# facebookresearch/mbrl-lib

Hardware: AMD Instinct MI355X
Metric: candidate-steps/sec (pop×particles×horizon / plan) per CEM iter; plans/sec (higher is better)
Workload: dtype f32

## Files before the change

mbrl-lib_amd/csrc/cem.hpp:

```cpp
#pragma once
#include <type_traits>

#include "common.hpp"

namespace hipets {

struct CemDev {
    int n_env;
    int pop, H, A, D;
    int K;
    float alpha, one_minus_alpha;
    int return_mean, clipped, unbiased;
    const float* totals = nullptr;
    int P = 0;
    const int* elite_in = nullptr;
};

__device__ __forceinline__ float philox_trunc_normal(uint32_t idx_lo, uint32_t idx_hi, uint64_t seed, uint64_t stream) {
    for (uint32_t attempt = 0; attempt < 64; ++attempt) {
        const Philox4 r = philox4x32_10(idx_lo, idx_hi, attempt, (uint32_t)stream, (uint32_t)seed,
                                        (uint32_t)(seed >> 32) ^ (uint32_t)(stream >> 32) ^ 0x5EED5EEDu);
        float n0, n1, n2, n3;
        box_muller(r.x, r.y, n0, n1);
        if (fabsf(n0) <= 2.0f) return n0;
        if (fabsf(n1) <= 2.0f) return n1;
        box_muller(r.z, r.w, n2, n3);
        if (fabsf(n2) <= 2.0f) return n2;
        if (fabsf(n3) <= 2.0f) return n3;
    }
    return 0.0f;
}

__device__ __forceinline__ float philox_normal(uint32_t idx_lo, uint32_t idx_hi, uint64_t seed, uint64_t stream) {
    const Philox4 r = philox4x32_10(idx_lo, idx_hi, 0u, (uint32_t)stream, (uint32_t)seed,
                                    (uint32_t)(seed >> 32) ^ (uint32_t)(stream >> 32) ^ 0x5EED5EEDu);
    float n0, n1;
    box_muller(r.x, r.y, n0, n1);
    return n0;
}

__global__ void cem_sample_kernel(const CemDev p, const float* __restrict__ mu, const float* __restrict__ disp,
                                  const float* __restrict__ lower, const float* __restrict__ upper,
                                  const float* __restrict__ z_in, unsigned long long seed, unsigned long long stream,
                                  float* __restrict__ population) {
    const long long i = (long long)blockIdx.x * blockDim.x + threadIdx.x;
    if (i >= (long long)p.n_env * p.pop * p.D) return;
    const int d = (int)(i % p.D);
    const int env = (int)(i / ((long long)p.pop * p.D));
    const float m = mu[env * p.D + d], v = disp[env * p.D + d], lb = lower[d], ub = upper[d];
    float x;
    if (p.clipped) {
        const float z = z_in ? z_in[i] : philox_normal((uint32_t)i, (uint32_t)(i >> 32), seed, stream);
        x = m + v * z;
        x = x > lb ? x : lb;
        x = x < ub ? x : ub;
    } else {
        const float lbd = (m - lb) / 2.0f, ubd = (ub - m) / 2.0f;
        const float mv = fminf(lbd * lbd, ubd * ubd);
        const float cv = fminf(mv, v);
        const float z = z_in ? z_in[i] : philox_trunc_normal((uint32_t)i, (uint32_t)(i >> 32), seed, stream);
        x = z * sqrtf(cv) + m;
    }
    population[i] = x;
}

#ifndef HIPETS_REFIT_SKIP
#define HIPETS_REFIT_SKIP 0
#endif
constexpr int kRefitThreads = 1024;
constexpr int kMaxPop = 8192;
constexpr int kRefitScratchBytes = 12288;
constexpr int kSelectMaxK = 1024;
constexpr int kRankSortMax = 640;

__global__ __launch_bounds__(kRefitThreads) void cem_refit_kernel(const CemDev p, float* values, const float* population, float* mu,
                                                                 float* disp, float* best_value, float* best_solution,
                                                                 int* elite_idx_out) {
    extern __shared__ __attribute__((aligned(16))) char smem[];
    {
        const int env = blockIdx.y;
        values += (size_t)env * p.pop;
        if (p.totals && !(HIPETS_REFIT_SKIP & 1)) {
            const float* tot = p.totals + (size_t)env * p.pop * p.P;
            for (int i = threadIdx.x; i < p.pop; i += kRefitThreads) {
                float s = 0.f;
                for (int q0 = 0; q0 < p.P; q0 += 8) {
                    float tv[8];
#pragma unroll
                    for (int u = 0; u < 8; ++u) tv[u] = tot[(size_t)i * p.P + min(q0 + u, p.P - 1)];
#pragma unroll
                    for (int u = 0; u < 8; ++u)
                        if (q0 + u < p.P) s += tv[u];
                }
                values[i] = s / (float)p.P;
            }
        }
        population += (size_t)env * p.pop * p.D;
        mu += (size_t)env * p.D;
        disp += (size_t)env * p.D;
        best_value += env;
        best_solution += (size_t)env * p.D;
        if (elite_idx_out) elite_idx_out += (size_t)env * p.K;
    }
    const int* const elite_in = p.elite_in ? p.elite_in + (size_t)blockIdx.y * p.K : nullptr;
    int n2 = 1;
    while (n2 < p.pop) n2 <<= 1;
    float* key = reinterpret_cast<float*>(smem);
    int* idx = reinterpret_cast<int*>(smem + (size_t)n2 * 4);
    const int tid = threadIdx.x;
    for (int i = tid; i < n2; i += kRefitThreads) {
        float v = -INFINITY;
        if (i < p.pop) {
            v = values[i];
            if (v != v) { v = -1e-10f; values[i] = v; }
        }
        key[i] = v;
        idx[i] = i < p.pop ? i : 0x7FFFFFFF;
    }
    __syncthreads();
    if (elite_in) {
        auto in_range = [&](const int e) { return e < 0 ? 0 : (e >= p.pop ? p.pop - 1 : e); };
        const float top_key = key[in_range(elite_in[0])];
        __syncthreads();
        for (int k = tid; k < p.K; k += kRefitThreads) idx[k] = in_range(elite_in[k]);
        if (tid == 0) key[0] = top_key;
        __syncthreads();
    } else if (HIPETS_REFIT_SKIP & 2) {
    } else if (p.pop <= kRankSortMax) {
        for (int i = tid; i < p.pop; i += kRefitThreads) {
            const float ki = key[i];
            int rank = 0;
#pragma unroll 8
            for (int j = 0; j < i; ++j) rank += key[j] >= ki;
#pragma unroll 8
            for (int j = i + 1; j < p.pop; ++j) rank += key[j] > ki;
            idx[i] = rank;
        }
        __syncthreads();
        int* pos = reinterpret_cast<int*>(smem + (size_t)n2 * 8);
        for (int i = tid; i < p.pop; i += kRefitThreads) pos[idx[i]] = i;
        __syncthreads();
        float top_key = key[pos[0]];
        __syncthreads();
        for (int i = tid; i < p.pop; i += kRefitThreads) idx[i] = pos[i];
        if (tid == 0) key[0] = top_key;
        __syncthreads();
    } else if (p.K <= kSelectMaxK) {
        int* hist = reinterpret_cast<int*>(smem + (size_t)n2 * 8);
        int* ctl = hist + 256;
        int* elist = ctl + 8;
        float* ekey = reinterpret_cast<float*>(elist + kSelectMaxK);
        auto okey = [](float v) {
            const unsigned u = __float_as_uint(v + 0.0f);
            return (u & 0x80000000u) ? ~u : (u | 0x80000000u);
        };
        if (tid == 0) { ctl[0] = 0; ctl[1] = 0; ctl[2] = p.K; ctl[3] = 0; }
        for (int pass = 3; pass >= 0; --pass) {
            for (int b = tid; b < 256; b += kRefitThreads) hist[b] = 0;
            __syncthreads();
            const unsigned prefix = (unsigned)ctl[0], mask = (unsigned)ctl[1];
            for (int i = tid; i < p.pop; i += kRefitThreads) {
                const unsigned u = okey(key[i]);
                if ((u & mask) == prefix) atomicAdd(&hist[(u >> (8 * pass)) & 255u], 1);
            }
            __syncthreads();
            if (tid < 64) {
                const int h0 = hist[4 * tid], h1 = hist[4 * tid + 1], h2 = hist[4 * tid + 2], h3 = hist[4 * tid + 3];
                const int mine = h0 + h1 + h2 + h3;
                int above = mine;
#pragma unroll
                for (int d = 1; d < 64; d <<= 1) {
                    const int o = __shfl_down(above, d, 64);
                    if (tid + d < 64) above += o;
                }
                const int need = ctl[2];
                const int higher = above - mine;
                if (higher < need && need <= above) {
                    int n = need - higher, b = 4 * tid + 3;
                    if (n > h3) { n -= h3; b = 4 * tid + 2;
                        if (n > h2) { n -= h2; b = 4 * tid + 1;
                            if (n > h1) { n -= h1; b = 4 * tid; } } }
                    ctl[0] = (int)(prefix | ((unsigned)b << (8 * pass)));
                    ctl[1] = (int)(mask | (255u << (8 * pass)));
                    ctl[2] = n;
                }
            }
            __syncthreads();
        }
        const unsigned T = (unsigned)ctl[0];
        const int need_eq = ctl[2];
        const bool all_eq = hist[T & 255u] == need_eq;
        for (int i = tid; i < p.pop; i += kRefitThreads) {
            const unsigned u = okey(key[i]);
            bool elite = u > T || (u == T && all_eq);
            if (u == T && !all_eq) {
                int before = 0;
                for (int j = 0; j < i; ++j) before += okey(key[j]) == T;
                elite = before < need_eq;
            }
            if (elite) {
                const int slot = atomicAdd(&ctl[3], 1);
                elist[slot] = i;
                ekey[slot] = key[i];
            }
        }
        __syncthreads();
        int my_pos = -1, my_id = 0;
        float my_key = 0.f;
        if (tid < p.K) {
            my_id = elist[tid];
            my_key = ekey[tid];
            int rank = 0;
            for (int f = 0; f < p.K; ++f) {
                const float kf = ekey[f];
                rank += (kf > my_key) || (kf == my_key && elist[f] < my_id);
            }
            my_pos = rank;
        }
        __syncthreads();
        if (my_pos >= 0) idx[my_pos] = my_id;
        if (my_pos == 0) key[0] = my_key;
        __syncthreads();
    } else
    for (int k = 2; k <= n2; k <<= 1) {
        for (int j = k >> 1; j > 0; j >>= 1) {
            for (int i = tid; i < n2; i += kRefitThreads) {
                const int ixj = i ^ j;
                if (ixj > i) {
                    const float ka = key[i], kb = key[ixj];
                    const int ia = idx[i], ib = idx[ixj];
                    const bool a_first = (ka > kb) || (ka == kb && ia < ib);
                    const bool up = (i & k) == 0;
                    if (up ? !a_first : a_first) {
                        key[i] = kb; key[ixj] = ka;
                        idx[i] = ib; idx[ixj] = ia;
                    }
                }
            }
            __syncthreads();
        }
    }
    if (elite_idx_out && blockIdx.x == 0)
        for (int k = tid; k < p.K; k += kRefitThreads) elite_idx_out[k] = idx[k];

    const float top = key[0];
    const bool improved = blockIdx.x == 0 && top > best_value[0];
    const int top_i = idx[0];
    __syncthreads();

    double* red = reinterpret_cast<double*>(smem + (size_t)n2 * 8);
    const int nb = (int)gridDim.x, bx = (int)blockIdx.x;
    const int Dslice = (((p.D + nb - 1) / nb + 63) / 64) * 64;
    const int d_lo = bx * Dslice, d_hi = min(p.D, d_lo + Dslice);
    int parts = kRefitThreads / Dslice;
    parts = parts < 1 ? 1 : (parts > 8 ? 8 : parts);
    const int G = kRefitThreads / parts;
    const int part = tid / G, dloc = tid % G;
    const int nu = (p.K + parts - 1) / parts;
    auto sweep = [&](const int base, auto nu_tag, auto hold_tag) __attribute__((always_inline)) {
        constexpr int NU = decltype(nu_tag)::value;
        constexpr bool HOLD = decltype(hold_tag)::value;
        const int d = base + dloc;
        const bool live = d < d_hi && part < parts;
        float mu_old = 0.f, disp_old = 0.f;
        float xv[NU];
        double s = 0.0;
        if (live) {
            if (part == 0) { mu_old = mu[d]; disp_old = disp[d]; }
            for (int k0 = part; k0 < (HOLD ? part + 1 : p.K); k0 += parts * NU) {
#pragma unroll
                for (int u = 0; u < NU; ++u) xv[u] = population[(size_t)idx[min(k0 + u * parts, p.K - 1)] * p.D + d];
#pragma unroll
                for (int u = 0; u < NU; ++u)
                    if (k0 + u * parts < p.K) s += (double)xv[u];
            }
        }
        red[tid] = s;
        __syncthreads();
        double mean = 0.0;
        if (live) {
            for (int q = 0; q < parts; ++q) mean += red[q * G + dloc];
            mean /= (double)p.K;
        }
        __syncthreads();
        double ss = 0.0;
        if (live) {
            for (int k0 = part; k0 < (HOLD ? part + 1 : p.K); k0 += parts * NU) {
                if constexpr (!HOLD) {
#pragma unroll
                    for (int u = 0; u < NU; ++u) xv[u] = population[(size_t)idx[min(k0 + u * parts, p.K - 1)] * p.D + d];
                }
#pragma unroll
                for (int u = 0; u < NU; ++u)
                    if (k0 + u * parts < p.K) {
                        const double dv = (double)xv[u] - mean;
                        ss += dv * dv;
                    }
            }
        }
        red[tid] = ss;
        __syncthreads();
        if (live && part == 0) {
            double var = 0.0;
            for (int q = 0; q < parts; ++q) var += red[q * G + dloc];
            var /= (double)(p.unbiased ? (p.K - 1) : p.K);
            const float new_mu = (float)mean;
            const float new_disp = p.clipped ? (float)sqrt(var) : (float)var;
            mu[d] = p.alpha * mu_old + p.one_minus_alpha * new_mu;
            disp[d] = p.alpha * disp_old + p.one_minus_alpha * new_disp;
        }
        __syncthreads();
    };
    constexpr int kBestHold = 4;
    float best_row[kBestHold];
    const bool best_held = p.D <= kBestHold * kRefitThreads;
    if (improved && best_held) {
#pragma unroll
        for (int u = 0; u < kBestHold; ++u) best_row[u] = population[(size_t)top_i * p.D + min(tid + u * kRefitThreads, p.D - 1)];
    }
    for (int base = d_lo; base < ((HIPETS_REFIT_SKIP & 4) ? d_lo : d_hi); base += G) {
        using T = std::true_type;
        using F = std::false_type;
        if (nu <= 2) sweep(base, std::integral_constant<int, 2>{}, T{});
        else if (nu <= 4) sweep(base, std::integral_constant<int, 4>{}, T{});
        else if (nu <= 8) sweep(base, std::integral_constant<int, 8>{}, T{});
        else if (nu <= 16) sweep(base, std::integral_constant<int, 16>{}, T{});
        else sweep(base, std::integral_constant<int, 16>{}, F{});
    }
    if (improved) {
        if (best_held) {
#pragma unroll
            for (int u = 0; u < kBestHold; ++u)
                if (tid + u * kRefitThreads < p.D) best_solution[tid + u * kRefitThreads] = best_row[u];
        } else {
            for (int d = tid; d < p.D; d += kRefitThreads) best_solution[d] = population[(size_t)top_i * p.D + d];
        }
        if (tid == 0) best_value[0] = top;
    }
}

inline int refit_blocks(const int D) { return D <= 128 ? 1 : (D + 127) / 128 > 8 ? 8 : (D + 127) / 128; }

__global__ void cem_init_kernel(const CemDev p, const float* x0, const float* lower, const float* upper, float* mu,
                                float* disp, float* best_value) {
    const int i = blockIdx.x * blockDim.x + threadIdx.x;
    if (i < p.n_env * p.D) {
        const int d = i % p.D;
        mu[i] = x0[i];
        const float w = upper[d] - lower[d];
        disp[i] = p.clipped ? 1.0f : (w * w) / 16.0f;
    }
    if (i < p.n_env) best_value[i] = -INFINITY;
}

}
```

mbrl-lib_amd/csrc/plan.hip:

```cpp
#include <algorithm>
#include <cmath>
#include <vector>

#include "engine.hpp"
#include "lds_optin.hpp"
#include "optim.hpp"

using namespace hipets;

namespace {

int launch_mppi_sample(int n_env, int pop, int H, int A, float beta, const float* mean, const float* past_action, const float* lower, const float* upper,
                       const float* z, uint64_t seed, uint64_t stream_id, float* population, hipStream_t st) {
    const long long npop = (long long)n_env * pop;
    const long long D = (long long)H * A;
    if (D <= kMppiSampleMaxD) {
        const int G = mppi_sample_group(npop, (int)D);
        hipLaunchKernelGGL(mppi_sample_staged_kernel, dim3((unsigned)((npop + G - 1) / G)), dim3(kMppiSampleThreads), (size_t)G * D * 4, st, n_env, pop, H, A, G, beta,
                           mean, past_action, lower, upper, z, (unsigned long long)seed, (unsigned long long)stream_id, population);
    } else {
        const long long n = npop * A;
        hipLaunchKernelGGL(mppi_sample_kernel, dim3((unsigned)((n + 255) / 256)), dim3(256), 0, st, n_env, pop, H, A, beta, mean, past_action, lower, upper, z,
                           (unsigned long long)seed, (unsigned long long)stream_id, population);
    }
    HCHECK(hipGetLastError());
    return 0;
}

int launch_mppi_update(hipets_engine* e, int n_env, int pop, int D, float gamma, float* values, const float* population, float* mean, hipStream_t st) {
    static LdsOptIn once[2];
    HCHECK(full_lds_once(once[0], reinterpret_cast<const void*>(&mppi_update_kernel<kMppiTileMax / 16>), (int)e->lds_max));
    HCHECK(full_lds_once(once[1], reinterpret_cast<const void*>(&mppi_update_kernel<kMppiTileMax / 32>), (int)e->lds_max));
    const int tile_c = mppi_update_tile(pop, e->lds_max);
    const dim3 grid(mppi_update_blocks(D), n_env);
    if (tile_c == kMppiTileMax)
        hipLaunchKernelGGL(mppi_update_kernel<kMppiTileMax / 16>, grid, dim3(kMppiThreads), mppi_update_smem(pop, tile_c), st, pop, D, gamma, values, population, mean);
    else
        hipLaunchKernelGGL(mppi_update_kernel<kMppiTileMax / 32>, grid, dim3(kMppiThreads), mppi_update_smem(pop, tile_c), st, pop, D, gamma, values, population, mean);
    HCHECK(hipGetLastError());
    return 0;
}

int plan_prologue(hipets_engine* e, const float* s0, int n_env, int H, int iters, uint64_t seed, uint64_t first_stream, hipStream_t st) {
    const ModelDev& md = e->md;
    if (e->s0.ensure((size_t)n_env * md.obs_dim * 4)) return 1;
    if (stage_h2d(e, e->s0.p, s0, (size_t)n_env * md.obs_dim * 4, st)) return 1;
    return plan_step_keys(e, H, iters, seed, first_stream, st);
}

inline void shard_bounds(int pop, int world, int r, int* lo, int* hi) {
    const int base = pop / world, extra = pop % world;
    *lo = r * base + std::min(r, extra);
    *hi = *lo + base + (r < extra ? 1 : 0);
}

int trace_iter(hipets_engine* e, int i, int rows, size_t nd, const float* population, const float* values, const float* mu,
               const float* disp, hipStream_t st, int n_env = 1) {
    if (!e->has_trace) return 0;
    const hipets_plan_trace& t = e->trace;
    if (rows > t.max_rows) return fail("plan trace: iteration %d evaluates %d candidates, trace buffers hold %d", i, rows, t.max_rows);
    const size_t ne = (size_t)n_env;
    if (t.populations && population)
        HCHECK(hipMemcpyAsync(t.populations + (size_t)i * t.max_rows * nd, population, (size_t)rows * nd * 4, hipMemcpyDeviceToDevice, st));
    if (t.values && values) HCHECK(hipMemcpyAsync(t.values + (size_t)i * t.max_rows, values, (size_t)rows * 4, hipMemcpyDeviceToDevice, st));
    if (t.mus && mu) HCHECK(hipMemcpyAsync(t.mus + (size_t)i * ne * nd, mu, ne * nd * 4, hipMemcpyDeviceToDevice, st));
    if (t.dispersions && disp) HCHECK(hipMemcpyAsync(t.dispersions + (size_t)i * ne * nd, disp, ne * nd * 4, hipMemcpyDeviceToDevice, st));
    return 0;
}

CemDev make_cem(const hipets_cem_params* p, int n_env = 1) {
    CemDev c{};
    c.n_env = n_env;
    c.pop = p->population_size;
    c.H = p->horizon;
    c.A = p->act_dim;
    c.D = p->horizon * p->act_dim;
    c.K = p->elite_num;
    c.alpha = (float)p->alpha;
    c.one_minus_alpha = (float)(1.0 - (double)p->alpha);
    c.return_mean = p->return_mean_elites;
    c.clipped = p->clipped_normal;
    c.unbiased = p->unbiased_var;
    return c;
}
// ... 27 lines not shown
    const int world = e->comm_world, rank = e->comm_rank;
    int lo, hi;
    shard_bounds(rows, world, rank, &lo, &hi);
    const int width = (rows + world - 1) / world;
    const size_t nd = (size_t)H * e->md.act_dim;
    float* shard_out = world == 1 ? e->values.as<float>() : e->shard_values.as<float>();
    if (le->ok()) le->note(rollout_impl(e, population + (size_t)lo * nd, nullptr, hi - lo, H, P, ro, shard_out, stream));
    if (world > 1) {
        hipStream_t st = reinterpret_cast<hipStream_t>(stream);
        if (comm_all_gather(e, (size_t)width, st)) return 1;
        if (le->ok()) le->note(comm_unpad_shards(e, rows, width, st));
    }
    return 0;
}

struct PlanObjective {
    enum Kind { ENSEMBLE, SHARDED, PLANET } kind = ENSEMBLE;
    const float* s0 = nullptr;
    const float* latent0 = nullptr;
    const float* belief0 = nullptr;

    bool is_planet() const { return kind == PLANET; }
    bool is_sharded() const { return kind == SHARDED; }
    uint64_t rollout_seed(const hipets_engine* e, uint64_t seed) const {
        return seed + (is_sharded() ? (uint64_t)e->comm_rank : 0ull) * 0x9E3779B97F4A7C15ull;
    }
    size_t shard_width(const hipets_engine* e, int max_rows) const { return (size_t)((max_rows + e->comm_world - 1) / e->comm_world); }
    int reserve_shards(hipets_engine* e, int max_rows) const {
        if (!is_sharded()) return 0;
        const size_t width = shard_width(e, max_rows);
        return e->shard_values.ensure(width * 4) || e->gathered.ensure((size_t)e->comm_world * width * 4);
    }
    int clear_padding(hipets_engine* e, int max_rows, hipStream_t st) const {
        if (is_sharded()) HCHECK(hipMemsetAsync(e->shard_values.p, 0, shard_width(e, max_rows) * 4, st));
        return 0;
    }
    void refit_from_totals(hipets_engine* e, CemDev* c, int P) const {
        if (is_sharded()) return;
        c->totals = e->totals.as<float>();
        c->P = P;
    }
    int evaluate(hipets_engine* e, const float* population, int rows, int H, int P, const hipets_rollout_opts* ro, float* returns,
                 void* stream, LocalErr& le) const {
        if (is_sharded()) return sharded_evaluate(e, population, rows, H, P, ro, stream, &le);
        if (!le.ok()) return 0;
        if (!is_planet()) {
            le.note(rollout_impl(e, population, nullptr, rows, H, P, ro, returns, stream));
            return 0;
        }
        hipets_planet_opts po{};
        po.seed = ro->seed;
        po.stream_id = ro->stream_id;
        po.n_env = ro->n_env;
        le.note(planet_rollout_impl(e, population, latent0, belief0, rows, H, P, &po, returns, reinterpret_cast<hipStream_t>(stream)));
        return 0;
    }
};
PlanObjective ensemble_objective(const float* s0, PlanObjective::Kind kind = PlanObjective::ENSEMBLE) {
    PlanObjective o;
    o.kind = kind;
    o.s0 = s0;
    return o;
}
PlanObjective planet_objective(const float* latent0, const float* belief0) {
    PlanObjective o;
    o.kind = PlanObjective::PLANET;
    o.latent0 = latent0;
    o.belief0 = belief0;
    return o;
}

int check_plan(const hipets_engine* e, const PlanObjective& obj, bool args, int A, int n_env, int P) {
    const bool planet = obj.is_planet();
    if (planet && !(e && e->has_planet)) return fail("engine has no PlaNet model (call hipets_planet_set_model)");
    if (!planet && !(e && e->has_model)) return fail("engine has no model (call hipets_set_model)");
    if (!args || (planet ? !(obj.latent0 && obj.belief0) : !obj.s0)) return fail("null argument");
    if (planet && A != e->pd.action) return fail("act_dim %d != model action_size %d", A, e->pd.action);
    if (!planet && A != e->md.act_dim) return fail("act_dim %d != model act_dim %d", A, e->md.act_dim);
    if (n_env < 1 || n_env > 4096) return fail("n_env %d outside [1, 4096]", n_env);
    if (planet && P < 1) return fail("bad pop/horizon/particles");
    return 0;
}

int launch_cem_refit(const CemDev& c, float* values, const float* population, float* mu, float* disp, float* best_value, float* best_solution,
                     int* elite_idx, hipStream_t st) {
    int n2 = 1;
    while (n2 < c.pop) n2 <<= 1;
    hipLaunchKernelGGL(cem_refit_kernel, dim3(refit_blocks(c.D), c.n_env), dim3(kRefitThreads), (size_t)n2 * 8 + kRefitScratchBytes, st, c, values,
                       population, mu, disp, best_value, best_solution, elite_idx);
    HCHECK(hipGetLastError());
    return 0;
}

struct PlanLoop {
    int n_env, H, P, iters;
    uint64_t first_stream, stream_stride, rollout_stream;
    const float* population;
    float* returns;
};
template <class Prologue, class Rows, class Sample, class Refit>
int run_plan(hipets_engine* e, const PlanObjective& obj, const PlanLoop& pl, uint64_t seed, void* stream, Prologue prologue, Rows rows, Sample sample,
             Refit refit) {
    hipets_rollout_opts ro{};
    ro.mode = e->plan_mode;
    ro.seed = obj.rollout_seed(e, seed);
    ro.n_env = pl.n_env;
    const bool carry_on = obj.is_sharded();
    LocalErr le;
    le.note(prologue(ro.seed));
    for (int i = 0; i < pl.iters && (carry_on || le.ok()); ++i) {
        const uint64_t sid = (pl.first_stream + (uint64_t)i) * pl.stream_stride;
        if (le.ok()) le.note(sample(i, sid));
        ro.stream_id = sid + pl.rollout_stream;
        if (obj.evaluate(e, pl.population, rows(i), pl.H, pl.P, &ro, pl.returns, stream, le)) return 1;
        if (le.ok()) le.note(refit(i));
    }
    return le.report();
}

int plan_cem_impl(hipets_engine* e, const hipets_cem_params* p, int32_t n_env, const float* x0, const float* lower, const float* upper,
                  const PlanObjective& obj, int32_t P, uint64_t seed, uint64_t plan_id, float* out, void* stream) {
    if (check_cem(p) || check_plan(e, obj, x0 && lower && upper && out, p->act_dim, n_env, P)) return 1;
    if (obj.is_sharded() && check_shards(e, p->population_size, P)) return 1;
    hipStream_t st = reinterpret_cast<hipStream_t>(stream);
    HCHECK(hipSetDevice(e->device));
    ENTER_STREAM(e, st);
    const CemDev c = make_cem(p, n_env);
    const size_t nd = (size_t)n_env * c.D, npop = (size_t)n_env * c.pop;
    if (e->mu.ensure(nd * 4) || e->disp.ensure(nd * 4) || e->best_solution.ensure(nd * 4) || e->best_value.ensure((size_t)n_env * 4 + 16) ||
        e->population.ensure(npop * c.D * 4) || e->values.ensure(npop * 4) || obj.reserve_shards(e, c.pop))
        return 1;
    const int iters = p->num_iterations;
    const PlanLoop pl{n_env, c.H, P, iters, plan_id * (uint64_t)iters, 1, 0, e->population.as<float>(), nullptr};
    auto prologue = [&](uint64_t rollout_seed) -> int {
        if (obj.clear_padding(e, c.pop, st)) return 1;
        hipLaunchKernelGGL(cem_init_kernel, dim3((unsigned)((nd + 255) / 256)), dim3(256), 0, st, c, x0, lower, upper, e->mu.as<float>(),
                           e->disp.as<float>(), e->best_value.as<float>());
        HCHECK(hipGetLastError());
        HCHECK(hipMemsetAsync(e->best_solution.p, 0, nd * 4, st));
        return obj.is_planet() ? 0 : plan_prologue(e, obj.s0, n_env, c.H, iters, rollout_seed, pl.first_stream, st);
    };
    auto sample = [&](int, uint64_t sid) -> int {
        const long long n = (long long)npop * c.D;
        hipLaunchKernelGGL(cem_sample_kernel, dim3((unsigned)((n + 255) / 256)), dim3(256), 0, st, c, e->mu.as<float>(), e->disp.as<float>(),
                           lower, upper, (const float*)nullptr, (unsigned long long)seed, (unsigned long long)sid, e->population.as<float>());
        HCHECK(hipGetLastError());
        return 0;
    };
    auto refit = [&](int i) -> int {
        int* eidx = (e->has_trace && e->trace.elite_idx) ? e->trace.elite_idx + (size_t)i * n_env * c.K : nullptr;
        CemDev cr = c;
        obj.refit_from_totals(e, &cr, P);
        if (launch_cem_refit(cr, e->values.as<float>(), e->population.as<float>(), e->mu.as<float>(), e->disp.as<float>(), e->best_value.as<float>(),
                             e->best_solution.as<float>(), eidx, st))
            return 1;
        return trace_iter(e, i, (int)npop, (size_t)c.D, e->population.as<float>(), e->values.as<float>(), e->mu.as<float>(), e->disp.as<float>(), st, n_env);
    };
    if (run_plan(e, obj, pl, seed, stream, prologue, [&](int) { return (int)npop; }, sample, refit)) return 1;
    HCHECK(hipMemcpyAsync(out, p->return_mean_elites ? e->mu.p : e->best_solution.p, nd * 4, hipMemcpyDeviceToDevice, st));
    return 0;
}

int plan_mppi_impl(hipets_engine* e, int32_t pop, int32_t H, int32_t A, int32_t num_iterations, double gamma, double beta, int32_t n_env,
                   float* mean, const float* lower, const float* upper, const PlanObjective& obj, int32_t P, uint64_t seed, uint64_t plan_id,
                   void* stream) {
    if (check_plan(e, obj, mean && lower && upper, A, n_env, P)) return 1;
    if (pop < 1 || pop > 12000) return fail("population_size %d outside [1, 12000]", pop);
    if (H < 1 || num_iterations < 0) return fail("bad horizon/num_iterations");
    if (obj.is_sharded() && check_shards(e, pop, P)) return 1;
    hipStream_t st = reinterpret_cast<hipStream_t>(stream);
    HCHECK(hipSetDevice(e->device));
    ENTER_STREAM(e, st);
    const size_t nd = (size_t)H * A, npop = (size_t)n_env * pop;
    if (e->mu.ensure(n_env * nd * 4) || e->past_action.ensure((size_t)n_env * A * 4) || e->population.ensure(npop * nd * 4) ||
        e->values.ensure(npop * 4) || obj.reserve_shards(e, pop))
        return 1;
    const PlanLoop pl{n_env, H, P, num_iterations, plan_id * (uint64_t)num_iterations, 1, 0, e->population.as<float>(), e->values.as<float>()};
    auto prologue = [&](uint64_t rollout_seed) -> int {
        if (obj.clear_padding(e, pop, st)) return 1;
        HCHECK(hipMemcpyAsync(e->mu.p, mean, n_env * nd * 4, hipMemcpyDeviceToDevice, st));
        hipLaunchKernelGGL(mppi_shift_kernel, dim3((unsigned)((n_env * nd + 255) / 256)), dim3(256), 0, st, n_env, H, A, e->mu.as<float>(), mean,
                           e->past_action.as<float>());
        HCHECK(hipGetLastError());
        return obj.is_planet() ? 0 : plan_prologue(e, obj.s0, n_env, H, num_iterations, rollout_seed, pl.first_stream, st);
    };
    auto sample = [&](int, uint64_t sid) -> int {
        return launch_mppi_sample(n_env, pop, H, A, (float)beta, mean, e->past_action.as<float>(), lower, upper, nullptr, seed, sid,
                                  e->population.as<float>(), st);
    };
    auto update = [&](int k) -> int {
        if (launch_mppi_update(e, n_env, pop, (int)nd, (float)gamma, e->values.as<float>(), e->population.as<float>(), mean, st)) return 1;
        return trace_iter(e, k, (int)npop, nd, e->population.as<float>(), e->values.as<float>(), mean, nullptr, st, n_env);
    };
    return run_plan(e, obj, pl, seed, stream, prologue, [&](int) { return (int)npop; }, sample, update);
}

int plan_icem_impl(hipets_engine* e, const hipets_icem_params* p, int32_t n_env, const float* x0, const float* lower, const float* upper,
                   float* elite, int32_t has_elite, const int32_t* keep_idx, const PlanObjective& obj, int32_t P, uint64_t seed, uint64_t plan_id,
                   float* out, void* stream) {
    if (check_plan(e, obj, p && x0 && lower && upper && elite && out, p ? p->act_dim : 0, n_env, P)) return 1;
    if (p->horizon < 2 || p->horizon > kMaxHorizon) return fail("iCEM horizon %d outside [2, %d]", p->horizon, kMaxHorizon);
    const int K = p->elite_num, keep = p->keep_elite_size, iters = p->num_iterations, H = p->horizon, A = p->act_dim;
    if (K < 1 || keep < 0 || keep > K) return fail("elite_num %d / keep_elite_size %d invalid", K, keep);
    if (p->population_size < 1 || iters < 0 || !(p->population_decay_factor > 0.0)) return fail("bad iCEM parameters");
    std::vector<int> sizes(iters), rows_of(iters);
    int max_rows = 1;
    for (int i = 0, he = has_elite; i < iters; ++i, he = 1) {
        int n = (int)std::ceil(std::fmax((double)p->population_size * std::pow(p->population_decay_factor, -(double)i), 2.0 * K));
        const int m = p->population_size_module;
        if (m > 0 && n % m) n += m - n % m;
        sizes[i] = n;
        if (n + keep > kMaxPop) return fail("iCEM iteration %d evaluates %d candidates (max %d)", i, n + keep, kMaxPop);
        rows_of[i] = n + (he ? ((i == iters - 1 && i != 0) ? 1 : keep) : 0);
        if (K > rows_of[i]) return fail("elite_num %d invalid", K);
        max_rows = std::max(max_rows, n + keep);
        if (obj.is_sharded() && check_shards(e, rows_of[i], P)) return 1;
    }
    hipStream_t st = reinterpret_cast<hipStream_t>(stream);
    HCHECK(hipSetDevice(e->device));
    ENTER_STREAM(e, st);
    const size_t nd = (size_t)H * A, ne = (size_t)n_env;
    if (e->mu.ensure(ne * nd * 4) || e->disp.ensure(ne * nd * 4) || e->best_solution.ensure(ne * nd * 4) || e->best_value.ensure(ne * 4 + 16) ||
        e->population.ensure(ne * max_rows * nd * 4) || e->values.ensure(ne * max_rows * 4) ||
        e->kept.ensure(ne * std::max(keep, 1) * nd * 4) || e->elite_idx.ensure(ne * K * 4) || e->keep_idx.ensure(ne * std::max(keep, 1) * 4) ||
        (!obj.is_planet() && e->s0.ensure(ne * e->md.obs_dim * 4)) || obj.reserve_shards(e, max_rows))
        return 1;
    hipets_cem_params cp{};
    cp.population_size = std::max(K, 1);
    cp.horizon = H;
    cp.act_dim = A;
    cp.num_iterations = iters;
    cp.elite_num = K;
    cp.alpha = p->alpha;
    cp.return_mean_elites = p->return_mean_elites;
    cp.clipped_normal = 0;
    cp.unbiased_var = 0;
    float* popbuf = e->population.as<float>();
    const PlanLoop pl{n_env, H, P, iters, plan_id * (uint64_t)iters, 4, 3, popbuf, nullptr};
    auto prologue = [&](uint64_t) -> int {
        if (obj.clear_padding(e, max_rows, st)) return 1;
        hipLaunchKernelGGL(cem_init_kernel, dim3((unsigned)((ne * nd + 255) / 256)), dim3(256), 0, st, make_cem(&cp, n_env), x0, lower, upper,
                           e->mu.as<float>(), e->disp.as<float>(), e->best_value.as<float>());
        HCHECK(hipGetLastError());
        HCHECK(hipMemsetAsync(e->best_solution.p, 0, ne * nd * 4, st));
        return obj.is_planet() ? 0 : stage_h2d(e, e->s0.p, obj.s0, ne * e->md.obs_dim * 4, st);
    };
    auto sample = [&](int i, uint64_t sid) -> int {
        const int n = sizes[i], rows = rows_of[i], extra = rows - n;
        launch_icem_sample(st, n_env, rows, n, H, A, (float)p->colored_noise_exponent, e->mu.as<float>(), e->disp.as<float>(), lower, upper,
                           (const float*)nullptr, (unsigned long long)seed, (unsigned long long)sid, popbuf);
        HCHECK(hipGetLastError());
        if (!extra) return 0;
        float* tail = popbuf + (size_t)n * nd;
        if (i == iters - 1 && i != 0) {
            hipLaunchKernelGGL(icem_append_mu_kernel, dim3((unsigned)((ne * nd + 255) / 256)), dim3(256), 0, st, n_env, rows, n, (int)nd,
                               e->mu.as<float>(), popbuf);
            HCHECK(hipGetLastError());
            return 0;
        }
        const int32_t* kidx = keep_idx ? keep_idx + (size_t)i * n_env * keep : e->keep_idx.as<int32_t>();
        if (!keep_idx) {
            hipLaunchKernelGGL(icem_keep_select_kernel, dim3(n_env), dim3(256), (size_t)K * 8, st, K, keep, (unsigned long long)seed,
                               (unsigned long long)(sid + 2), e->keep_idx.as<int32_t>());
            HCHECK(hipGetLastError());
        }
        const long long ng = (long long)keep * nd;
        if (i == 0) {
            hipLaunchKernelGGL(gather_rows_kernel, dim3((unsigned)((ng + 255) / 256), n_env), dim3(256), 0, st, keep, (int)nd, elite, kidx,
                               e->kept.as<float>(), (long long)K * nd, (long long)keep * nd);
            HCHECK(hipGetLastError());
            hipLaunchKernelGGL(icem_shift_kernel, dim3((unsigned)((ne * ng + 255) / 256)), dim3(256), 0, st, n_env, rows, keep, H, A,
                               e->kept.as<float>(), e->mu.as<float>(), e->disp.as<float>(), (const float*)nullptr,
                               (unsigned long long)seed, (unsigned long long)(sid + 1), tail);
            HCHECK(hipGetLastError());
        } else {
            hipLaunchKernelGGL(gather_rows_kernel, dim3((unsigned)((ng + 255) / 256), n_env), dim3(256), 0, st, keep, (int)nd, elite, kidx,
                               tail, (long long)K * nd, (long long)rows * nd);
            HCHECK(hipGetLastError());
        }
        return 0;
    };
    auto refit = [&](int i) -> int {
        const int rows = rows_of[i];
        cp.population_size = rows;
        if (check_cem(&cp)) return 1;
        CemDev cr = make_cem(&cp, n_env);
        obj.refit_from_totals(e, &cr, P);
        if (launch_cem_refit(cr, e->values.as<float>(), popbuf, e->mu.as<float>(), e->disp.as<float>(), e->best_value.as<float>(),
                             e->best_solution.as<float>(), e->elite_idx.as<int>(), st))
            return 1;
        const long long nk = (long long)K * nd;
        hipLaunchKernelGGL(gather_rows_kernel, dim3((unsigned)((nk + 255) / 256), n_env), dim3(256), 0, st, K, (int)nd, popbuf, e->elite_idx.as<int32_t>(),
                           elite, (long long)rows * nd, (long long)K * nd);
        HCHECK(hipGetLastError());
        if (trace_iter(e, i, n_env * rows, nd, popbuf, e->values.as<float>(), e->mu.as<float>(), e->disp.as<float>(), st, n_env)) return 1;
        if (e->has_trace && e->trace.elite_idx)
            HCHECK(hipMemcpyAsync(e->trace.elite_idx + (size_t)i * n_env * K, e->elite_idx.p, ne * K * 4, hipMemcpyDeviceToDevice, st));
        return 0;
    };
    if (run_plan(e, obj, pl, seed, stream, prologue, [&](int i) { return n_env * rows_of[i]; }, sample, refit)) return 1;
    HCHECK(hipMemcpyAsync(out, p->return_mean_elites ? e->mu.p : e->best_solution.p, ne * nd * 4, hipMemcpyDeviceToDevice, st));
    return 0;
}

}

extern "C" {

int hipets_cem_sample(hipets_engine* e, const hipets_cem_params* p, const float* mu, const float* dispersion,
                      const float* lower, const float* upper, const float* z, uint64_t seed, uint64_t stream_id,
                      float* population, void* stream) {
    if (!e) return fail("null engine");
    if (check_cem(p)) return 1;
    if (!mu || !dispersion || !lower || !upper || !population) return fail("null argument");
    HCHECK(hipSetDevice(e->device));
    const CemDev c = make_cem(p);
    const long long n = (long long)c.pop * c.D;
    hipLaunchKernelGGL(cem_sample_kernel, dim3((unsigned)((n + 255) / 256)), dim3(256), 0, reinterpret_cast<hipStream_t>(stream), c,
                       mu, dispersion, lower, upper, z, (unsigned long long)seed, (unsigned long long)stream_id, population);
    HCHECK(hipGetLastError());
    return 0;
}

int hipets_cem_refit(hipets_engine* e, const hipets_cem_params* p, float* values, const float* population, float* mu,
                     float* dispersion, float* best_value, float* best_solution, int32_t* elite_idx, void* stream) {
    if (!e) return fail("null engine");
    if (check_cem(p)) return 1;
// ... 152 lines not shown
```

Baseline: 290.6 million.

## Fuse CEM refit with next-iteration sampling and wave-ballot rank sort

Adds a fused boundary variant of the CEM refit kernel. It computes particle means inline, updates mu/disp and the best solution per D-slice, then samples the next population, or writes the output on the last iteration, in the same launch. This removes the separate sample kernel, the final memcpy and the memset. The small-population rank sort is replaced with wave-level ballot/popcount counting over register-held keys. best_value is now double-buffered across iterations so blocks can read the previous best without racing. The cost is a wider grid with some redundant per-block sorting and more complex indexing.

```diff
diff --git a/mbrl-lib_amd/csrc/cem.hpp b/mbrl-lib_amd/csrc/cem.hpp
--- a/mbrl-lib_amd/csrc/cem.hpp
+++ b/mbrl-lib_amd/csrc/cem.hpp
@@ -14,6 +14,16 @@
     const float* totals = nullptr;
     int P = 0;
     const int* elite_in = nullptr;
+    int slice = 0, parts = 1;
+};
+
+struct CemNext {
+    const float* lower = nullptr;
+    const float* upper = nullptr;
+    unsigned long long seed = 0, stream = 0;
+    float* next_population = nullptr;
+    float* out = nullptr;
+    const float* best_in = nullptr;
 };
 
 __device__ __forceinline__ float philox_trunc_normal(uint32_t idx_lo, uint32_t idx_hi, uint64_t seed, uint64_t stream) {
@@ -39,15 +49,8 @@
     return n0;
 }
 
-__global__ void cem_sample_kernel(const CemDev p, const float* __restrict__ mu, const float* __restrict__ disp,
-                                  const float* __restrict__ lower, const float* __restrict__ upper,
-                                  const float* __restrict__ z_in, unsigned long long seed, unsigned long long stream,
-                                  float* __restrict__ population) {
-    const long long i = (long long)blockIdx.x * blockDim.x + threadIdx.x;
-    if (i >= (long long)p.n_env * p.pop * p.D) return;
-    const int d = (int)(i % p.D);
-    const int env = (int)(i / ((long long)p.pop * p.D));
-    const float m = mu[env * p.D + d], v = disp[env * p.D + d], lb = lower[d], ub = upper[d];
+__device__ __forceinline__ float cem_sample_one(const CemDev& p, const long long i, const float m, const float v, const float lb, const float ub,
+                                                const float* __restrict__ z_in, unsigned long long seed, unsigned long long stream) {
     float x;
     if (p.clipped) {
         const float z = z_in ? z_in[i] : philox_normal((uint32_t)i, (uint32_t)(i >> 32), seed, stream);
@@ -61,6 +64,18 @@
         const float z = z_in ? z_in[i] : philox_trunc_normal((uint32_t)i, (uint32_t)(i >> 32), seed, stream);
         x = z * sqrtf(cv) + m;
     }
+    return x;
+}
+
+__global__ void cem_sample_kernel(const CemDev p, const float* __restrict__ mu, const float* __restrict__ disp,
+                                  const float* __restrict__ lower, const float* __restrict__ upper,
+                                  const float* __restrict__ z_in, unsigned long long seed, unsigned long long stream,
+                                  float* __restrict__ population) {
+    const long long i = (long long)blockIdx.x * blockDim.x + threadIdx.x;
+    if (i >= (long long)p.n_env * p.pop * p.D) return;
+    const int d = (int)(i % p.D);
+    const int env = (int)(i / ((long long)p.pop * p.D));
+    const float x = cem_sample_one(p, i, mu[env * p.D + d], disp[env * p.D + d], lower[d], upper[d], z_in, seed, stream);
     population[i] = x;
 }
 
@@ -73,28 +88,42 @@
 constexpr int kSelectMaxK = 1024;
 constexpr int kRankSortMax = 640;
 
+__device__ __forceinline__ float particle_mean(const float* __restrict__ row, const int P) {
+    float s = 0.f;
+    if ((P & 3) == 0) {
+        const float4* r4 = reinterpret_cast<const float4*>(row);
+        const int nq = P >> 2;
+        for (int q0 = 0; q0 < nq; q0 += 8) {
+            float4 tv[8];
+#pragma unroll
+            for (int u = 0; u < 8; ++u) tv[u] = r4[min(q0 + u, nq - 1)];
+#pragma unroll
+            for (int u = 0; u < 8; ++u)
+                if (q0 + u < nq) { s += tv[u].x; s += tv[u].y; s += tv[u].z; s += tv[u].w; }
+        }
+    } else {
+        for (int q0 = 0; q0 < P; q0 += 8) {
+            float tv[8];
+#pragma unroll
+            for (int u = 0; u < 8; ++u) tv[u] = row[min(q0 + u, P - 1)];
+#pragma unroll
+            for (int u = 0; u < 8; ++u)
+                if (q0 + u < P) s += tv[u];
+        }
+    }
+    return s / (float)P;
+}
+
+template <bool FUSED>
 __global__ __launch_bounds__(kRefitThreads) void cem_refit_kernel(const CemDev p, float* values, const float* population, float* mu,
                                                                  float* disp, float* best_value, float* best_solution,
-                                                                 int* elite_idx_out) {
+                                                                 int* elite_idx_out, const CemNext nx) {
     extern __shared__ __attribute__((aligned(16))) char smem[];
+    const float* tot = nullptr;
     {
         const int env = blockIdx.y;
         values += (size_t)env * p.pop;
-        if (p.totals && !(HIPETS_REFIT_SKIP & 1)) {
-            const float* tot = p.totals + (size_t)env * p.pop * p.P;
-            for (int i = threadIdx.x; i < p.pop; i += kRefitThreads) {
-                float s = 0.f;
-                for (int q0 = 0; q0 < p.P; q0 += 8) {
-                    float tv[8];
-#pragma unroll
-                    for (int u = 0; u < 8; ++u) tv[u] = tot[(size_t)i * p.P + min(q0 + u, p.P - 1)];
-#pragma unroll
-                    for (int u = 0; u < 8; ++u)
-                        if (q0 + u < p.P) s += tv[u];
-                }
-                values[i] = s / (float)p.P;
-            }
-        }
+        if (p.totals && !(HIPETS_REFIT_SKIP & 1)) tot = p.totals + (size_t)env * p.pop * p.P;
         population += (size_t)env * p.pop * p.D;
         mu += (size_t)env * p.D;
         disp += (size_t)env * p.D;
@@ -111,8 +140,10 @@
     for (int i = tid; i < n2; i += kRefitThreads) {
         float v = -INFINITY;
         if (i < p.pop) {
-            v = values[i];
-            if (v != v) { v = -1e-10f; values[i] = v; }
+            bool fresh = tot != nullptr;
+            v = tot ? particle_mean(tot + (size_t)i * p.P, p.P) : values[i];
+            if (v != v) { v = -1e-10f; fresh = true; }
+            if (fresh && blockIdx.x == 0) values[i] = v;
         }
         key[i] = v;
         idx[i] = i < p.pop ? i : 0x7FFFFFFF;
@@ -127,18 +158,32 @@
         __syncthreads();
     } else if (HIPETS_REFIT_SKIP & 2) {
     } else if (p.pop <= kRankSortMax) {
-        for (int i = tid; i < p.pop; i += kRefitThreads) {
-            const float ki = key[i];
+        constexpr int kBlocks = kRankSortMax / 64;
+        static_assert(kRankSortMax % 64 == 0 && kRankSortMax / (kRefitThreads / 64) <= 64, "rank counting: a wave's elements fit its lanes");
+        const int lane = tid & 63, wave = tid >> 6, nblk = (p.pop + 63) >> 6;
+        float kj[kBlocks];
+#pragma unroll
+        for (int r = 0; r < kBlocks; ++r) kj[r] = 64 * r + lane < n2 ? key[64 * r + lane] : -INFINITY;
+        const int mine = __float_as_int(key[min(wave + (kRefitThreads / 64) * lane, n2 - 1)]);
+        int* pos = reinterpret_cast<int*>(smem + (size_t)n2 * 8);
+        for (int i = wave, t = 0; i < p.pop; i += kRefitThreads / 64, ++t) {
+            const float ki = __int_as_float(__builtin_amdgcn_readlane(mine, t));
+            const int bi = i >> 6;
             int rank = 0;
-#pragma unroll 8
-            for (int j = 0; j < i; ++j) rank += key[j] >= ki;
-#pragma unroll 8
-            for (int j = i + 1; j < p.pop; ++j) rank += key[j] > ki;
-            idx[i] = rank;
-        }
-        __syncthreads();
-        int* pos = reinterpret_cast<int*>(smem + (size_t)n2 * 8);
-        for (int i = tid; i < p.pop; i += kRefitThreads) pos[idx[i]] = i;
+#pragma unroll
+            for (int r = 0; r < kBlocks; ++r) {
+                if (r >= nblk) break;
+                unsigned long long m;
+                if (r < bi) m = __ballot(kj[r] >= ki);
+                else if (r > bi) m = __ballot(kj[r] > ki);
+                else {
+                    const unsigned long long below = (1ull << (i & 63)) - 1ull;
+                    m = (__ballot(kj[r] >= ki) & below) | (__ballot(kj[r] > ki) & ~below);
+                }
+                rank += __popcll(m);
+            }
+            if (lane == 0) pos[rank] = i;
+        }
         __syncthreads();
         float top_key = key[pos[0]];
         __syncthreads();
@@ -244,16 +289,16 @@
         for (int k = tid; k < p.K; k += kRefitThreads) elite_idx_out[k] = idx[k];
 
     const float top = key[0];
-    const bool improved = blockIdx.x == 0 && top > best_value[0];
+    const float best_old = FUSED ? nx.best_in[blockIdx.y] : (blockIdx.x == 0 ? best_value[0] : INFINITY);
+    const bool improved = top > best_old;
     const int top_i = idx[0];
     __syncthreads();
 
     double* red = reinterpret_cast<double*>(smem + (size_t)n2 * 8);
-    const int nb = (int)gridDim.x, bx = (int)blockIdx.x;
-    const int Dslice = (((p.D + nb - 1) / nb + 63) / 64) * 64;
-    const int d_lo = bx * Dslice, d_hi = min(p.D, d_lo + Dslice);
-    int parts = kRefitThreads / Dslice;
-    parts = parts < 1 ? 1 : (parts > 8 ? 8 : parts);
+    const int bx = (int)blockIdx.x;
+    const int d_lo = min(p.D, bx * p.slice), d_hi = min(p.D, d_lo + p.slice);
+    const int parts = p.parts;
+    float* fresh = reinterpret_cast<float*>(smem + (size_t)n2 * 8 + kRefitThreads * 8);
     const int G = kRefitThreads / parts;
     const int part = tid / G, dloc = tid % G;
     const int nu = (p.K + parts - 1) / parts;
@@ -306,17 +351,23 @@
             var /= (double)(p.unbiased ? (p.K - 1) : p.K);
             const float new_mu = (float)mean;
             const float new_disp = p.clipped ? (float)sqrt(var) : (float)var;
-            mu[d] = p.alpha * mu_old + p.one_minus_alpha * new_mu;
-            disp[d] = p.alpha * disp_old + p.one_minus_alpha * new_disp;
+            const float mu_d = p.alpha * mu_old + p.one_minus_alpha * new_mu;
+            const float disp_d = p.alpha * disp_old + p.one_minus_alpha * new_disp;
+            mu[d] = mu_d;
+            disp[d] = disp_d;
+            if constexpr (FUSED) { fresh[2 * (d - d_lo)] = mu_d; fresh[2 * (d - d_lo) + 1] = disp_d; }
         }
         __syncthreads();
     };
     constexpr int kBestHold = 4;
     float best_row[kBestHold];
-    const bool best_held = p.D <= kBestHold * kRefitThreads;
+    const bool best_held = FUSED || p.D <= kBestHold * kRefitThreads;
     if (improved && best_held) {
-#pragma unroll
-        for (int u = 0; u < kBestHold; ++u) best_row[u] = population[(size_t)top_i * p.D + min(tid + u * kRefitThreads, p.D - 1)];
+        if constexpr (FUSED) best_row[0] = population[(size_t)top_i * p.D + min(d_lo + tid, p.D - 1)];
+        else {
+#pragma unroll
+            for (int u = 0; u < kBestHold; ++u) best_row[u] = population[(size_t)top_i * p.D + min(tid + u * kRefitThreads, p.D - 1)];
+        }
     }
     for (int base = d_lo; base < ((HIPETS_REFIT_SKIP & 4) ? d_lo : d_hi); base += G) {
         using T = std::true_type;
@@ -327,7 +378,21 @@
         else if (nu <= 16) sweep(base, std::integral_constant<int, 16>{}, T{});
         else sweep(base, std::integral_constant<int, 16>{}, F{});
     }
-    if (improved) {
+    if constexpr (FUSED) {
+        const int W = d_hi - d_lo, env = (int)blockIdx.y;
+        if (improved && tid < W) best_solution[d_lo + tid] = best_row[0];
+        if (bx == 0 && tid == 0) best_value[0] = improved ? top : best_old;
+        if (nx.out && tid < W)
+            nx.out[(size_t)env * p.D + d_lo + tid] = p.return_mean ? fresh[2 * tid] : (improved ? best_row[0] : best_solution[d_lo + tid]);
+        if (nx.next_population) {
+            float* next = nx.next_population + (size_t)env * p.pop * p.D;
+            for (int e = tid; e < p.pop * W; e += kRefitThreads) {
+                const int c = e / W, dl = e - c * W, d = d_lo + dl;
+                const long long i = ((long long)env * p.pop + c) * p.D + d;
+                next[(size_t)c * p.D + d] = cem_sample_one(p, i, fresh[2 * dl], fresh[2 * dl + 1], nx.lower[d], nx.upper[d], nullptr, nx.seed, nx.stream);
+            }
+        }
+    } else if (improved) {
         if (best_held) {
 #pragma unroll
             for (int u = 0; u < kBestHold; ++u)
@@ -340,17 +405,32 @@
 }
 
 inline int refit_blocks(const int D) { return D <= 128 ? 1 : (D + 127) / 128 > 8 ? 8 : (D + 127) / 128; }
+inline int refit_slice(const int D) { return (((D + refit_blocks(D) - 1) / refit_blocks(D) + 63) / 64) * 64; }
+inline int refit_parts(const int D) {
+    const int parts = kRefitThreads / refit_slice(D);
+    return parts < 1 ? 1 : (parts > 8 ? 8 : parts);
+}
+constexpr int kBoundaryMaxSlice = 128;
+constexpr int kBoundaryWorkgroups = 256;
+static_assert(kRefitThreads * 8 + kBoundaryMaxSlice * 8 <= kRefitScratchBytes, "fused boundary: LDS behind the partial sums");
+inline int boundary_slice(const int D, const int n_env) {
+    const int per_env = kBoundaryWorkgroups / (n_env < 1 ? 1 : n_env) < 1 ? 1 : kBoundaryWorkgroups / (n_env < 1 ? 1 : n_env);
+    const int nb = D < per_env ? D : per_env;
+    const int s = (D + nb - 1) / nb;
+    return s > kBoundaryMaxSlice ? 0 : s;
+}
 
 __global__ void cem_init_kernel(const CemDev p, const float* x0, const float* lower, const float* upper, float* mu,
-                                float* disp, float* best_value) {
+                                float* disp, float* best_value, float* best_solution) {
     const int i = blockIdx.x * blockDim.x + threadIdx.x;
     if (i < p.n_env * p.D) {
         const int d = i % p.D;
         mu[i] = x0[i];
         const float w = upper[d] - lower[d];
         disp[i] = p.clipped ? 1.0f : (w * w) / 16.0f;
-    }
-    if (i < p.n_env) best_value[i] = -INFINITY;
-}
-
-}
+        best_solution[i] = 0.0f;
+    }
+    if (i < 2 * p.n_env) best_value[i] = -INFINITY;
+}
+
+}
diff --git a/mbrl-lib_amd/csrc/plan.hip b/mbrl-lib_amd/csrc/plan.hip
--- a/mbrl-lib_amd/csrc/plan.hip
+++ b/mbrl-lib_amd/csrc/plan.hip
@@ -1,5 +1,6 @@
 #include <algorithm>
 #include <cmath>
+#include <cstdlib>
 #include <vector>
 
 #include "engine.hpp"
@@ -193,12 +194,39 @@
     return 0;
 }
 
-int launch_cem_refit(const CemDev& c, float* values, const float* population, float* mu, float* disp, float* best_value, float* best_solution,
+int launch_cem_refit(CemDev c, float* values, const float* population, float* mu, float* disp, float* best_value, float* best_solution,
                      int* elite_idx, hipStream_t st) {
     int n2 = 1;
     while (n2 < c.pop) n2 <<= 1;
-    hipLaunchKernelGGL(cem_refit_kernel, dim3(refit_blocks(c.D), c.n_env), dim3(kRefitThreads), (size_t)n2 * 8 + kRefitScratchBytes, st, c, values,
-                       population, mu, disp, best_value, best_solution, elite_idx);
+    c.slice = refit_slice(c.D);
+    c.parts = refit_parts(c.D);
+    hipLaunchKernelGGL(cem_refit_kernel<false>, dim3(refit_blocks(c.D), c.n_env), dim3(kRefitThreads), (size_t)n2 * 8 + kRefitScratchBytes, st, c, values,
+                       population, mu, disp, best_value, best_solution, elite_idx, CemNext{});
+    HCHECK(hipGetLastError());
+    return 0;
+}
+
+int plan_boundary_slice(const int D, const int n_env) {
+    static const int forced = [] { const char* v = std::getenv("HIPETS_BOUNDARY_SLICE"); return v && v[0] ? std::atoi(v) : -1; }();
+    if (forced < 0) return boundary_slice(D, n_env);
+    return forced > kBoundaryMaxSlice ? kBoundaryMaxSlice : forced;
+}
+int launch_cem_boundary(CemDev c, int slice, float* values, const float* population, float* mu, float* disp, float* best_out, float* best_solution,
+                        int* elite_idx, const CemNext& nx, hipStream_t st) {
+    int n2 = 1;
+    while (n2 < c.pop) n2 <<= 1;
+    c.slice = slice;
+    c.parts = refit_parts(c.D);
+    hipLaunchKernelGGL(cem_refit_kernel<true>, dim3((c.D + c.slice - 1) / c.slice, c.n_env), dim3(kRefitThreads), (size_t)n2 * 8 + kRefitScratchBytes, st, c,
+                       values, population, mu, disp, best_out, best_solution, elite_idx, nx);
+    HCHECK(hipGetLastError());
+    return 0;
+}
+
+int launch_cem_init(hipets_engine* e, const CemDev& c, const float* x0, const float* lower, const float* upper, hipStream_t st) {
+    const size_t n = std::max((size_t)c.n_env * c.D, (size_t)2 * c.n_env);
+    hipLaunchKernelGGL(cem_init_kernel, dim3((unsigned)((n + 255) / 256)), dim3(256), 0, st, c, x0, lower, upper, e->mu.as<float>(), e->disp.as<float>(),
+                       e->best_value.as<float>(), e->best_solution.as<float>());
     HCHECK(hipGetLastError());
     return 0;
 }
@@ -238,20 +266,19 @@
     ENTER_STREAM(e, st);
     const CemDev c = make_cem(p, n_env);
     const size_t nd = (size_t)n_env * c.D, npop = (size_t)n_env * c.pop;
-    if (e->mu.ensure(nd * 4) || e->disp.ensure(nd * 4) || e->best_solution.ensure(nd * 4) || e->best_value.ensure((size_t)n_env * 4 + 16) ||
+    if (e->mu.ensure(nd * 4) || e->disp.ensure(nd * 4) || e->best_solution.ensure(nd * 4) || e->best_value.ensure((size_t)n_env * 8 + 16) ||
         e->population.ensure(npop * c.D * 4) || e->values.ensure(npop * 4) || obj.reserve_shards(e, c.pop))
         return 1;
     const int iters = p->num_iterations;
     const PlanLoop pl{n_env, c.H, P, iters, plan_id * (uint64_t)iters, 1, 0, e->population.as<float>(), nullptr};
     auto prologue = [&](uint64_t rollout_seed) -> int {
-        if (obj.clear_padding(e, c.pop, st)) return 1;
-        hipLaunchKernelGGL(cem_init_kernel, dim3((unsigned)((nd + 255) / 256)), dim3(256), 0, st, c, x0, lower, upper, e->mu.as<float>(),
-                           e->disp.as<float>(), e->best_value.as<float>());
-        HCHECK(hipGetLastError());
-        HCHECK(hipMemsetAsync(e->best_solution.p, 0, nd * 4, st));
+        if (obj.clear_padding(e, c.pop, st) || launch_cem_init(e, c, x0, lower, upper, st)) return 1;
         return obj.is_planet() ? 0 : plan_prologue(e, obj.s0, n_env, c.H, iters, rollout_seed, pl.first_stream, st);
     };
-    auto sample = [&](int, uint64_t sid) -> int {
+    const int slice = plan_boundary_slice(c.D, n_env);
+    const bool one_launch = slice > 0;
+    auto sample = [&](int i, uint64_t sid) -> int {
+        if (one_launch && i > 0) return 0;
         const long long n = (long long)npop * c.D;
         hipLaunchKernelGGL(cem_sample_kernel, dim3((unsigned)((n + 255) / 256)), dim3(256), 0, st, c, e->mu.as<float>(), e->disp.as<float>(),
                            lower, upper, (const float*)nullptr, (unsigned long long)seed, (unsigned long long)sid, e->population.as<float>());
@@ -262,13 +289,29 @@
         int* eidx = (e->has_trace && e->trace.elite_idx) ? e->trace.elite_idx + (size_t)i * n_env * c.K : nullptr;
         CemDev cr = c;
         obj.refit_from_totals(e, &cr, P);
-        if (launch_cem_refit(cr, e->values.as<float>(), e->population.as<float>(), e->mu.as<float>(), e->disp.as<float>(), e->best_value.as<float>(),
-                             e->best_solution.as<float>(), eidx, st))
+        if (!one_launch) {
+            if (launch_cem_refit(cr, e->values.as<float>(), e->population.as<float>(), e->mu.as<float>(), e->disp.as<float>(), e->best_value.as<float>(),
+                                 e->best_solution.as<float>(), eidx, st))
+                return 1;
+            return trace_iter(e, i, (int)npop, (size_t)c.D, e->population.as<float>(), e->values.as<float>(), e->mu.as<float>(), e->disp.as<float>(), st, n_env);
+        }
+        if (trace_iter(e, i, (int)npop, (size_t)c.D, e->population.as<float>(), nullptr, nullptr, nullptr, st, n_env)) return 1;
+        const bool last = i + 1 == iters;
+        CemNext nx;
+        nx.lower = lower;
+        nx.upper = upper;
+        nx.seed = seed;
+        nx.stream = (pl.first_stream + (uint64_t)i + 1) * pl.stream_stride;
+        nx.next_population = last ? nullptr : e->population.as<float>();
+        nx.out = last ? out : nullptr;
+        nx.best_in = e->best_value.as<float>() + (size_t)(i & 1) * n_env;
+        if (launch_cem_boundary(cr, slice, e->values.as<float>(), e->population.as<float>(), e->mu.as<float>(), e->disp.as<float>(),
+                                e->best_value.as<float>() + (size_t)((i + 1) & 1) * n_env, e->best_solution.as<float>(), eidx, nx, st))
             return 1;
-        return trace_iter(e, i, (int)npop, (size_t)c.D, e->population.as<float>(), e->values.as<float>(), e->mu.as<float>(), e->disp.as<float>(), st, n_env);
+        return trace_iter(e, i, (int)npop, (size_t)c.D, nullptr, e->values.as<float>(), e->mu.as<float>(), e->disp.as<float>(), st, n_env);
     };
     if (run_plan(e, obj, pl, seed, stream, prologue, [&](int) { return (int)npop; }, sample, refit)) return 1;
-    HCHECK(hipMemcpyAsync(out, p->return_mean_elites ? e->mu.p : e->best_solution.p, nd * 4, hipMemcpyDeviceToDevice, st));
+    if (!one_launch || iters < 1) HCHECK(hipMemcpyAsync(out, p->return_mean_elites ? e->mu.p : e->best_solution.p, nd * 4, hipMemcpyDeviceToDevice, st));
     return 0;
 }
 
@@ -331,7 +374,7 @@
     HCHECK(hipSetDevice(e->device));
     ENTER_STREAM(e, st);
     const size_t nd = (size_t)H * A, ne = (size_t)n_env;
-    if (e->mu.ensure(ne * nd * 4) || e->disp.ensure(ne * nd * 4) || e->best_solution.ensure(ne * nd * 4) || e->best_value.ensure(ne * 4 + 16) ||
+    if (e->mu.ensure(ne * nd * 4) || e->disp.ensure(ne * nd * 4) || e->best_solution.ensure(ne * nd * 4) || e->best_value.ensure(ne * 8 + 16) ||
         e->population.ensure(ne * max_rows * nd * 4) || e->values.ensure(ne * max_rows * 4) ||
         e->kept.ensure(ne * std::max(keep, 1) * nd * 4) || e->elite_idx.ensure(ne * K * 4) || e->keep_idx.ensure(ne * std::max(keep, 1) * 4) ||
         (!obj.is_planet() && e->s0.ensure(ne * e->md.obs_dim * 4)) || obj.reserve_shards(e, max_rows))
@@ -350,10 +393,7 @@
     const PlanLoop pl{n_env, H, P, iters, plan_id * (uint64_t)iters, 4, 3, popbuf, nullptr};
     auto prologue = [&](uint64_t) -> int {
         if (obj.clear_padding(e, max_rows, st)) return 1;
-        hipLaunchKernelGGL(cem_init_kernel, dim3((unsigned)((ne * nd + 255) / 256)), dim3(256), 0, st, make_cem(&cp, n_env), x0, lower, upper,
-                           e->mu.as<float>(), e->disp.as<float>(), e->best_value.as<float>());
-        HCHECK(hipGetLastError());
-        HCHECK(hipMemsetAsync(e->best_solution.p, 0, ne * nd * 4, st));
+        if (launch_cem_init(e, make_cem(&cp, n_env), x0, lower, upper, st)) return 1;
         return obj.is_planet() ? 0 : stage_h2d(e, e->s0.p, obj.s0, ne * e->md.obs_dim * 4, st);
     };
     auto sample = [&](int i, uint64_t sid) -> int {
diff --git a/profiles/critical_path_probe.py b/profiles/critical_path_probe.py
--- /dev/null
+++ b/profiles/critical_path_probe.py
@@ -0,0 +1,64 @@
+import argparse
+import json
+import os
+import statistics
+import sys
+import time
+
+ROOT = os.path.dirname(os.path.dirname(os.path.abspath(__file__)))
+sys.path[:0] = [ROOT, os.path.join(ROOT, "mbrl-lib_amd")]
+import numpy as np
+import torch
+
+import bench
+import hipets
+from hipets.planning import _BoundObjective
+
+ap = argparse.ArgumentParser()
+ap.add_argument("--label", default="this")
+ap.add_argument("--out", default=None)
+ap.add_argument("--blocks", type=int, default=3)
+ap.add_argument("--plans", type=int, default=60)
+args = ap.parse_args()
+
+dev = torch.device("cuda:0")
+eng = hipets.get_engine(dev)
+cases = {"cfg2_device": (dict(), 500, 20, 30), "cfg1_device": (dict(obs=4, act=1, ensemble=5, reward="cartpole", termination="cartpole"), 100, 5, 15)}
+run = {"lib": os.environ.get("HIPETS_LIB", "default")}
+for name, (mkw, pop, P, H) in cases.items():
+    spec = bench.synthetic_spec(dev, **mkw)
+    act, obs = spec.act_dim, spec.obs_dim
+    fn = hipets.make_eval_fn(spec, P, engine=eng, seed=0, mode="device")
+    opt = hipets.CEMOptimizer(5, 0.1, pop, [[-1.0] * act] * H, [[1.0] * act] * H, 0.1, dev, return_mean_elites=True, seed=0)
+    obj = _BoundObjective(fn, np.zeros(obs, np.float32))
+    x0 = torch.zeros(H, act, device=dev)
+    t0 = time.perf_counter()
+    while time.perf_counter() - t0 < 0.5:
+        opt.optimize(obj, x0=x0)
+        torch.cuda.synchronize()
+    wall, kern = [], []
+    for _ in range(args.blocks):
+        torch.cuda.synchronize()
+        t0 = time.perf_counter()
+        for _ in range(args.plans):
+            opt.optimize(obj, x0=x0)
+        torch.cuda.synchronize()
+        wall.append(1e3 * (time.perf_counter() - t0) / args.plans)
+        eng.timing_enable(True)
+        eng.timing_read(reset=True)
+        for _ in range(20):
+            opt.optimize(obj, x0=x0)
+        torch.cuda.synchronize()
+        n, ms = eng.timing_read(reset=True)
+        eng.timing_enable(False)
+        kern.append(ms / 20)
+    w, k = statistics.median(wall), statistics.median(kern)
+    run[name] = {"ms_per_plan_blocks": [round(x, 5) for x in wall], "ms_per_plan": w, "rollout_kernels_ms_per_plan": k,
+                 "outside_rollouts_us_per_plan": 1e3 * (w - k)}
+print(json.dumps(run))
+if args.out:
+    doc = json.load(open(args.out)) if os.path.exists(args.out) else {}
+    doc.setdefault("runs", {}).setdefault(args.label, []).append(run)
+    with open(args.out, "w") as f:
+        json.dump(doc, f, indent=1)
+        f.write("\n")
```

After: 284.5 million. -2.1%, worse.
